# UZ-SLAMLab/DefSLAM

Measured on AMD Instinct MI355X. Metric: SfT GN iters/sec (500-node mesh, 1k matches), higher is better.
Workload: dtype f64

## Files before the change

### defslam_amd/csrc/sft_batch.h

```cpp
#pragma once

#define SFTB_NW 8
#ifndef SFTB_LIN_NW
#define SFTB_LIN_NW 8
#endif
#ifndef SFTB_LIN_WAVES
#define SFTB_LIN_WAVES 2
#endif
#ifndef SFTB_TRIAL_WAVES
#define SFTB_TRIAL_WAVES 2
#endif

__device__ __forceinline__ void sftb_ctl_lds(char* smem, Ctl*& ctl, double*& red, double*& out, double*& panel) {
  ctl = reinterpret_cast<Ctl*>(smem);
  red = reinterpret_cast<double*>(smem + 512);
  out = red + 16 * 27 + 5;
  panel = out + 32;
}

__global__ __launch_bounds__(64 * SFTB_NW, 2) void sftb_init_kernel(const SftDev* __restrict__ probs, SftRun* __restrict__ runs, int* __restrict__ counters, int* __restrict__ lin_list, int tail_below) {
  const SftDev& P = probs[blockIdx.x];
  if (blockIdx.x == 0 && threadIdx.x == 0 && (int)gridDim.x <= tail_below) counters[6] = 1;
  init_state<64 * SFTB_NW>(P);
  if (threadIdx.x == 0) {
// ... 48 lines not shown
    const int b = __builtin_amdgcn_readfirstlane(next_b);
    if (b < 0) break;
    if (tid == 0) { nxt = fetch(); atomicAdd(&counters[9], 1); }
    sftb_lin_problem<NW>(probs[b], runs[b], ctl, red, out, panel);
  }
}

__global__ __launch_bounds__(64, 1) void sftb_factor_kernel(const SftDev* __restrict__ probs, SftRun* __restrict__ runs, int* __restrict__ counters, int B) {
  extern __shared__ __attribute__((aligned(16))) char smem[];
  lds_double* lds = to_lds(reinterpret_cast<double*>(smem));
  const int lane = threadIdx.x;
  if (counters[6]) return;
  for (int i = lane; i < WV_LDS_DOUBLES; i += 64) lds[i] = 0.0;
  if (blockIdx.x == 0 && lane == 0) { counters[2] = 0; counters[3] = 0; }
  WvPrev Q;
  Q.Lg = nullptr; Q.Linv = nullptr; Q.x = nullptr; Q.nT = 0; Q.active = 0; Q.xb = 0.0;
  int n_done = 0;
  while (true) {
    int b = 0;
    if (lane == 0) b = atomicAdd(&counters[1], 1);
    b = __builtin_amdgcn_readfirstlane(b);
    if (b >= B) break;
    if (runs[b].state != SFTB_TRIAL) continue;
    const SftDev& P = probs[b];
    const double lambda = runs[b].lambda;
    double xcam;
    const int ok = wv_factor(P, lambda, lambda, lds, Q, xcam);
    if (lane == 0) runs[b].fact_ok = ok;
    Q = wv_prev_of(P, ok, xcam, lane);
    n_done++;
  }
  int lane_now;
  asm volatile("v_mbcnt_lo_u32_b32 %0, -1, 0\n\tv_mbcnt_hi_u32_b32 %0, -1, %0" : "=v"(lane_now));
  if (Q.active) wv_backsub_now(Q, lane_now);
  if (lane_now == 0 && n_done) atomicAdd(&counters[8], n_done);
}

template <int NW>
__device__ __forceinline__ int sftb_trial_problem(const SftDev& P, SftRun& R, Ctl* ctl, double* red, double* out, double* panel, int* counters, int* lin_list, int b) {
  constexpr int NT = 64 * NW;
  const int tid = threadIdx.x;
  const int Dn = P.Dn;
  const int Dnp = ((Dn + NB - 1) / NB) * NB;
  const int ok = R.fact_ok;
  const double lam = R.lambda;
  const bool in_lds = P.lds_class >= 1;
  if (!in_lds)
    for (int i = tid; i < 3 * P.n; i += NT) {
      const double v = P.xyz[i];
      P.xyz_bak[i] = v;
      const int a = P.act[i / 3];
      if (a >= 0) P.xyz[i] = v + P.x[3 * a + (i % 3)];
    }
  if (tid < 7) R.pose_bak[tid] = P.pose[tid];
  __syncthreads();
  if (tid == 0) pose_oplus(P.pose, P.x + Dnp);
  double sc = 0.0;
  for (int r = tid; r < Dn; r += NT) { const double xv = P.x[r]; sc += xv * (lam * xv + P.Hbord[(size_t)6 * Dnp + r]); }
  if (tid < 6) { const double xv = P.x[Dnp + tid]; sc += xv * (lam * xv + P.Hcorner[42 + tid]); }
  __syncthreads();
  block_sum<1>(&sc, red, out);
  const double scale = out[0];
  __syncthreads();
  const auto staged = asm_records<NW, 1>(P, panel);
  const double chi_new = in_lds ? eval_edges<false, 1>(P, ctl, red, out, staged, P.x)
                                : eval_edges<false, 0>(P, ctl, red, out, asm_records<NW, 0>(P, panel));
  if (tid == 0) {
// ... 133 lines not shown
```

### defslam_amd/csrc/sft_wave.h

```cpp
#pragma once

#if defined(WV_STEP_TRACE) && defined(DSH_LAB)
#define WV_T_DECL long long wv_tr[9] = {0, 0, 0, 0, 0, 0, 0, 0, 0}, wv_tl = clock64()
#define WV_T(e) do { const long long t__ = clock64(); wv_tr[e] += t__ - wv_tl; wv_tl = t__; } while (0)
#define WV_T_ARG , long long (&wv_tr)[9], long long& wv_tl
#define WV_T_PASS , wv_tr, wv_tl
#define WV_T_DUMP(P) do { if ((threadIdx.x & 63) == 0) for (int e__ = 0; e__ < 9; e__++) (P).dbg[40 + e__] = (double)wv_tr[e__]; } while (0)
#else
#define WV_T_DECL do {} while (0)
#define WV_T(e) do {} while (0)
#define WV_T_ARG
#define WV_T_PASS
#define WV_T_DUMP(P) do {} while (0)
#endif

__host__ __device__ constexpr int wv_phys(int r, int d) {
  return d == 0 ? r : (d <= 3 ? 8 * d + r : (d == 4 ? 32 + (r & 3) : 8 * (8 - d) + ((r + 8 - d) & 7)));
}
constexpr int WV_AGPR_TILES = 32;
constexpr int WV_L_WIN = 0;
constexpr int WV_L_BORD = 1024;
constexpr int WV_L_WSCR = 2048;
constexpr int WV_L_CN = 2336;
constexpr int WV_L_XRING = 2400;
constexpr int WV_L_LAND = 2528;
constexpr int WV_LDS_DOUBLES = WV_L_LAND + 10 * 256;
typedef double v2d_w __attribute__((ext_vector_type(2)));
#ifndef WV_DMA_AUX
#define WV_DMA_AUX 0
#endif
using lds_v2d = __attribute__((address_space(3))) v2d_w;

#define WV_NOP_MFMA_RESULT "s_nop 15\n\ts_nop 3"

template <int T>
__device__ __forceinline__ void wv_upd_agpr(const v4d& A, const v4d& B, int q0 = 0) {
  static_assert(T >= 0 && T < WV_AGPR_TILES, "accumulator tile");
#define WV_MF(q) asm volatile("v_mfma_f64_16x16x4_f64 a[%c0:%c1], %2, %3, a[%c0:%c1] neg:[1,0,0]" ::"i"(8 * T), "i"(8 * T + 7), "v"(A[q]), "v"(B[q]) : "memory")
  if (q0 <= 0) WV_MF(0);
  if (q0 <= 1) WV_MF(1);
  if (q0 <= 2) WV_MF(2);
  WV_MF(3);
#undef WV_MF
}
__device__ __forceinline__ void wv_upd_vgpr(v4d& C, const v4d& A, const v4d& B, int q0 = 0) {
#define WV_MF(q) asm volatile("v_mfma_f64_16x16x4_f64 %0, %1, %2, %0 neg:[1,0,0]" : "+v"(C) : "v"(A[q]), "v"(B[q]) : "memory")
  asm volatile("s_nop 1" : "+v"(C));
  if (q0 <= 0) WV_MF(0);
  if (q0 <= 1) WV_MF(1);
  if (q0 <= 2) WV_MF(2);
  WV_MF(3);
#undef WV_MF
}
template <int T>
__device__ __forceinline__ void wv_trsm_agpr(v4d& Y, const v4d& Wt) {
  asm volatile("v_mfma_f64_16x16x4_f64 %0, %1, a[%c5:%c6], 0\n\t"
               "v_mfma_f64_16x16x4_f64 %0, %2, a[%c7:%c8], %0\n\t"
               "v_mfma_f64_16x16x4_f64 %0, %3, a[%c9:%c10], %0\n\t"
               "v_mfma_f64_16x16x4_f64 %0, %4, a[%c11:%c12], %0"
               : "=&v"(Y)
               : "v"(Wt[0]), "v"(Wt[1]), "v"(Wt[2]), "v"(Wt[3]), "i"(8 * T), "i"(8 * T + 1), "i"(8 * T + 2), "i"(8 * T + 3), "i"(8 * T + 4), "i"(8 * T + 5),
                 "i"(8 * T + 6), "i"(8 * T + 7)
               : "memory");
}
__device__ __forceinline__ void wv_trsm_vgpr(v4d& Y, const v4d& Wt, const v4d& D, int q0 = 0) {
  if (q0 <= 0) {
    asm volatile("s_nop 1\n\t"
                 "v_mfma_f64_16x16x4_f64 %0, %1, %5, 0\n\t"
                 "v_mfma_f64_16x16x4_f64 %0, %2, %6, %0\n\t"
                 "v_mfma_f64_16x16x4_f64 %0, %3, %7, %0\n\t"
                 "v_mfma_f64_16x16x4_f64 %0, %4, %8, %0"
                 : "=&v"(Y)
                 : "v"(Wt[0]), "v"(Wt[1]), "v"(Wt[2]), "v"(Wt[3]), "v"(D[0]), "v"(D[1]), "v"(D[2]), "v"(D[3])
                 : "memory");
  } else {
    asm volatile("s_nop 1\n\tv_mfma_f64_16x16x4_f64 %0, %1, %2, 0" : "=&v"(Y) : "v"(Wt[3]), "v"(D[3]) : "memory");
    if (q0 <= 2) asm volatile("v_mfma_f64_16x16x4_f64 %0, %1, %2, %0" : "+v"(Y) : "v"(Wt[2]), "v"(D[2]) : "memory");
    if (q0 <= 1) asm volatile("v_mfma_f64_16x16x4_f64 %0, %1, %2, %0" : "+v"(Y) : "v"(Wt[1]), "v"(D[1]) : "memory");
  }
}
struct WvTri { double a[10]; };
__device__ __forceinline__ void wv_tri_load(const lds_double* wscr, int lane, WvTri& A) {
  const lds_double* p = wscr + (lane & 3) * 17 + (lane >> 4);
#pragma unroll
  for (int q = 0; q < 4; q++)
// ... 90 lines not shown
__device__ __forceinline__ void wv_bq_store(lds_double* tile, int lane, const WvB2& v) {
  reinterpret_cast<lds_v2d*>(tile)[lane] = (v2d_w){v.n0, v.n1};
}
__device__ __forceinline__ int wv_bo_lane(int lane) { return (lane & 0x30) | (lane & 3); }
__device__ __forceinline__ void wv_bo_load(const lds_double* tile, int lane, WvBO& o) {
  const lds_v2d* p = reinterpret_cast<const lds_v2d*>(tile) + wv_bo_lane(lane);
#pragma unroll
  for (int q = 0; q < 4; q++) { const v2d_w a = p[4 * q]; o.v[q][0] = a.x; o.v[q][1] = a.y; }
}
__device__ __forceinline__ void wv_upd_b4(WvB2& C, const v4d& A, const WvBO& B, int q0 = 0) {
#define WV_MF(q) asm volatile("v_mfma_f64_4x4x4_4b_f64 %0, %2, %3, %0 neg:[1,0,0]\n\tv_mfma_f64_4x4x4_4b_f64 %1, %2, %4, %1 neg:[1,0,0]" \
                              : "+v"(C.n0), "+v"(C.n1) : "v"(A[q]), "v"(B.v[q][0]), "v"(B.v[q][1]) : "memory")
  asm volatile("s_nop 1" : "+v"(C.n0), "+v"(C.n1));
  if (q0 <= 0) WV_MF(0);
  if (q0 <= 1) WV_MF(1);
  if (q0 <= 2) WV_MF(2);
  WV_MF(3);
#undef WV_MF
}
__device__ __forceinline__ void wv_trsm_b4(WvB2& Y, const v4d& Wt, const WvBO& B) {
  asm volatile("s_nop 1\n\t"
               "v_mfma_f64_4x4x4_4b_f64 %0, %2, %6, 0\n\t"
               "v_mfma_f64_4x4x4_4b_f64 %1, %2, %7, 0\n\t"
               "v_mfma_f64_4x4x4_4b_f64 %0, %3, %8, %0\n\t"
               "v_mfma_f64_4x4x4_4b_f64 %1, %3, %9, %1\n\t"
               "v_mfma_f64_4x4x4_4b_f64 %0, %4, %10, %0\n\t"
               "v_mfma_f64_4x4x4_4b_f64 %1, %4, %11, %1\n\t"
               "v_mfma_f64_4x4x4_4b_f64 %0, %5, %12, %0\n\t"
               "v_mfma_f64_4x4x4_4b_f64 %1, %5, %13, %1"
               : "=&v"(Y.n0), "=&v"(Y.n1)
               : "v"(Wt[0]), "v"(Wt[1]), "v"(Wt[2]), "v"(Wt[3]), "v"(B.v[0][0]), "v"(B.v[0][1]), "v"(B.v[1][0]), "v"(B.v[1][1]), "v"(B.v[2][0]), "v"(B.v[2][1]),
                 "v"(B.v[3][0]), "v"(B.v[3][1])
               : "memory");
}
__device__ __forceinline__ int wv_bstd_index(int lane) { return 2 * wv_bo_lane(lane) + ((lane >> 2) & 1); }

template <int CTRL>
__device__ __forceinline__ double wv_dpp_mov(double v) {
  const int lo = __builtin_amdgcn_mov_dpp(__double2loint(v), CTRL, 0xF, 0xF, false);
  const int hi = __builtin_amdgcn_mov_dpp(__double2hiint(v), CTRL, 0xF, 0xF, false);
  return __hiloint2double(hi, lo);
}

__device__ __forceinline__ bool wv_chol_inv(v4d& a, v4d& w) {
  const int lane = threadIdx.x & 63;
  const int g = lane >> 4, c = lane & 15;
  w = (v4d){(g == c) ? 1.0 : 0.0, (g + 4 == c) ? 1.0 : 0.0, (g + 8 == c) ? 1.0 : 0.0, (g + 12 == c) ? 1.0 : 0.0};
  double plast = 1.0;
#pragma unroll
  for (int J = 0; J < 4; J++) {
    const double aJ = a[J];
    const double sel = chol4_inverse_operand(aJ, J, g, c & 3, plast);
    const double wJ = w[J];
    double zw, lp;
    if (J < 3) {
      asm volatile("s_nop 1\n\t"
                   "v_mfma_f64_4x4x4_4b_f64 %0, %2, %3, 0\n\t"
                   "v_mfma_f64_4x4x4_4b_f64 %1, %2, %4, 0\n\t"
                   "s_nop 7"
                   : "=&v"(zw), "=&v"(lp)
                   : "v"(sel), "v"(wJ), "v"(aJ));
      const double nlp = -lp;
      const double below = (c >= 4 * J + 4) ? nlp : 0.0;
      asm volatile("s_nop 1\n\t"
                   "v_mfma_f64_16x16x4_f64 %0, %2, %3, %0\n\t"
                   "v_mfma_f64_16x16x4_f64 %1, %4, %5, %1\n\t" WV_NOP_MFMA_RESULT
                   : "+v"(a), "+v"(w)
                   : "v"(nlp), "v"(lp), "v"(below), "v"(zw));
      w[J] = zw;
    } else {
      asm volatile("s_nop 1\n\tv_mfma_f64_4x4x4_4b_f64 %0, %1, %2, 0\n\ts_nop 7" : "=&v"(zw) : "v"(sel), "v"(wJ));
      w[J] = zw;
    }
  }
// ... 54 lines not shown
};
__device__ __forceinline__ void wv_bs_request(const WvPrev& Q, int J, lds_double* land, int lane) {
  const unsigned voff = 16u * (unsigned)lane;
  const SFT_G char* col = reinterpret_cast<const SFT_G char*>(Q.Lg + ((size_t)J * (BT + 1)) * 256);
  const SFT_G char* w = reinterpret_cast<const SFT_G char*>(Q.Linv + (size_t)J * 256);
  const unsigned l0 = (unsigned)__builtin_amdgcn_readfirstlane((int)(size_t)land);
  asm volatile("s_mov_b32 m0, %2\n\ts_nop 0\n\t"
               "global_load_lds_dwordx4 %0, %1\n\t"
               "global_load_lds_dwordx4 %0, %1 offset:2048\n\t"
               "global_load_lds_dwordx4 %0, %1 offset:3072"
               :: "v"(voff), "s"(col), "s"(l0) : "memory", "m0");
#pragma unroll
  for (int grp = 1; grp < 5; grp++) {
    const SFT_G char* cg = col + 4096 * grp;
    const unsigned lg = l0 + 4096u * grp;
    if (grp < 4)
      asm volatile("s_mov_b32 m0, %2\n\ts_nop 0\n\t"
                   "global_load_lds_dwordx4 %0, %1\n\t"
                   "global_load_lds_dwordx4 %0, %1 offset:1024\n\t"
                   "global_load_lds_dwordx4 %0, %1 offset:2048\n\t"
                   "global_load_lds_dwordx4 %0, %1 offset:3072"
                   :: "v"(voff), "s"(cg), "s"(lg) : "memory", "m0");
    else
      asm volatile("s_mov_b32 m0, %2\n\ts_nop 0\n\t"
                   "global_load_lds_dwordx4 %0, %1\n\t"
                   "global_load_lds_dwordx4 %0, %1 offset:1024"
                   :: "v"(voff), "s"(cg), "s"(lg) : "memory", "m0");
  }
  asm volatile("s_mov_b32 m0, %2\n\ts_nop 0\n\t"
               "global_load_lds_dwordx4 %0, %1\n\t"
               "global_load_lds_dwordx4 %0, %1 offset:1024"
               :: "v"(voff), "s"(w), "s"(l0 + 18u * 1024u) : "memory", "m0");
}
__device__ __forceinline__ void wv_bs_column(const WvPrev& Q, int J, const lds_double* land, lds_double* xring, int lane) {
  const int c = lane & 15;
  const lds_v2d* t2 = reinterpret_cast<const lds_v2d*>(land) + 2 * lane;
  double s[4];
  {
    const lds_double* tb = land + wv_bstd_index(lane);
    s[0] = tb[0] * Q.xb; s[1] = tb[8] * Q.xb; s[2] = tb[16] * Q.xb; s[3] = tb[24] * Q.xb;
  }
#pragma unroll
  for (int d = 1; d <= 8; d++) {
    const double xr = xring[((J + d) & 7) * 16 + c];
    const v2d_w a = t2[128 * d], b = t2[128 * d + 1];
    s[0] = fma(a.x, xr, s[0]); s[1] = fma(a.y, xr, s[1]); s[2] = fma(b.x, xr, s[2]); s[3] = fma(b.y, xr, s[3]);
  }
#pragma unroll
  for (int q = 0; q < 4; q++) {
    s[q] += wv_dpp_mov<0x128>(s[q]);
    s[q] += wv_dpp_mov<0x124>(s[q]);
    s[q] += wv_dpp_mov<0x122>(s[q]);
    s[q] += wv_dpp_mov<0x121>(s[q]);
  }
  const v2d_w wa = t2[128 * 9], wb = t2[128 * 9 + 1];
  double p = wa.x * -s[0];
  p = fma(wa.y, -s[1], p); p = fma(wb.x, -s[2], p); p = fma(wb.y, -s[3], p);
  p = sum_rows(p);
  if (lane < TS) { xring[(J & 7) * 16 + lane] = p; Q.x[TS * J + lane] = p; }
}
__device__ __forceinline__ void wv_bs_step(const WvPrev& Q, int J, lds_double* lds, int lane) {
  wv_bs_column(Q, J, lds + WV_L_LAND, lds + WV_L_XRING, lane);
  asm volatile("s_waitcnt lgkmcnt(0)" ::: "memory");
  if (J >= 1) wv_bs_request(Q, J - 1, lds + WV_L_LAND, lane);
}
__device__ __forceinline__ void wv_bs_begin(const WvPrev& Q, lds_double* lds, int lane) {
  lds_double* xring = lds + WV_L_XRING;
  xring[lane] = 0.0; xring[64 + lane] = 0.0;
  wv_bs_request(Q, Q.nT - 1, lds + WV_L_LAND, lane);
}
__device__ __forceinline__ void wv_backsub_now(const WvPrev& Q, int lane) {
  const int c = lane & 15;
  (void)c;
  double xr[8];
#pragma unroll
  for (int s = 0; s < 8; s++) xr[s] = 0.0;
  struct Col { v4d t[10]; };
  auto fetch = [&](int J) -> Col {
    Col C;
    if (J >= 0) {
      const SFT_G double* col = Q.Lg + ((size_t)J * (BT + 1)) * 256 + 4 * lane;
#pragma unroll
      for (int i = 1; i <= 8; i++) C.t[i] = (J + i < Q.nT) ? *reinterpret_cast<const SFT_G v4d*>(col + 256 * i) : (v4d){0.0, 0.0, 0.0, 0.0};
      {
        const SFT_G double* tb = col - 4 * lane + wv_bstd_index(lane);
        C.t[0] = (v4d){tb[0], tb[8], tb[16], tb[24]};
      }
      C.t[9] = *reinterpret_cast<const SFT_G v4d*>(Q.Linv + (size_t)J * 256 + 4 * lane);
    } else {
#pragma unroll
      for (int i = 0; i < 10; i++) C.t[i] = (v4d){0.0, 0.0, 0.0, 0.0};
    }
    return C;
  };
  auto solve_col = [&](const Col& C, int J, auto phc) {
    constexpr int ph = decltype(phc)::value;
    double s[4];
#pragma unroll
    for (int q = 0; q < 4; q++) s[q] = C.t[0][q] * Q.xb;
#pragma unroll
    for (int dd = 1; dd <= 8; dd++)
#pragma unroll
      for (int q = 0; q < 4; q++) s[q] = fma(C.t[dd][q], xr[(ph + dd) & 7], s[q]);
#pragma unroll
    for (int q = 0; q < 4; q++) {
      s[q] += wv_dpp_mov<0x128>(s[q]);
      s[q] += wv_dpp_mov<0x124>(s[q]);
      s[q] += wv_dpp_mov<0x122>(s[q]);
      s[q] += wv_dpp_mov<0x121>(s[q]);
    }
    double p = C.t[9][0] * -s[0];
#pragma unroll
    for (int q = 1; q < 4; q++) p = fma(C.t[9][q], -s[q], p);
    p = sum_rows(p);
    xr[ph] = p;
    if (lane < TS) Q.x[TS * J + lane] = p;
  };
  int J = Q.nT - 1;
  Col c0 = fetch(J), c1 = fetch(J - 1);
#pragma unroll 1
  for (; J >= 0; J -= 2) {
    const Col n0 = fetch(J - 2), n1 = fetch(J - 3);
    switch (J & 7) {
      case 7: solve_col(c0, J, std::integral_constant<int, 7>{}); solve_col(c1, J - 1, std::integral_constant<int, 6>{}); break;
      case 5: solve_col(c0, J, std::integral_constant<int, 5>{}); solve_col(c1, J - 1, std::integral_constant<int, 4>{}); break;
      case 3: solve_col(c0, J, std::integral_constant<int, 3>{}); solve_col(c1, J - 1, std::integral_constant<int, 2>{}); break;
      default: solve_col(c0, J, std::integral_constant<int, 1>{}); solve_col(c1, J - 1, std::integral_constant<int, 0>{}); break;
    }
    c0 = n0; c1 = n1;
  }
}

struct WvState {
  v4d Y[9];
  WvB2 Yq;
  WvBO Yo;
  double corner;
  v4d araw;
  WvB2 bnext;
  WvRowList rl;
  unsigned al[4];
  unsigned off_lane, off_bord;
  int ok;
};

template <int PH, int I, int IEND>
__device__ __forceinline__ void wv_trsm_cols(WvState& S, const WvTri& Wt, int k, int nT, const v4d& D4, int lane) {
  if constexpr (I <= IEND) {
    (void)k; (void)nT;
    if constexpr (I == 4) {
      wv_trsm4_vgpr(S.Y[4], Wt, D4);
    } else {
      wv_trsm4_agpr<wv_phys((PH + I) & 7, I)>(S.Y[I], Wt);
    }
    wv_trsm_cols<PH, I + 1, IEND>(S, Wt, k, nT, D4, lane);
  }
}

__host__ __device__ constexpr int wv_tile_index(int I, int J) {
  int n = 0;
  for (int i = 1; i <= 7; i++)
    for (int j = 1; j <= i; j++) {
// ... 36 lines not shown
  }
}
template <int PH, bool TAIL, int I0, int I1>
__device__ __forceinline__ void wv_update_rows(const WvProb& W, WvState& S, int k, int nT, int q8, SFT_G double* col) {
  if constexpr (I0 <= I1) {
    wv_update_tiles<PH, TAIL, I0, 1>(W, S, k, nT, q8, col);
    wv_update_rows<PH, TAIL, I0 + 1, I1>(W, S, k, nT, q8, col);
  }
}
template <int PH, int T>
__device__ __forceinline__ lds_double* wv_task_tile(lds_double* lds) {
  if constexpr (T < 7) return lds + WV_L_BORD + 128 * ((PH + T + 1) & 7);
  else if constexpr (T < 10) return lds + WV_L_WIN + 256 * (wv_phys((PH + T - 2) & 7, 4) - WV_AGPR_TILES);
  else if constexpr (T == 10) return lds + WV_L_BORD + 128 * (PH & 7);
  else return lds + WV_L_WIN + 256 * (wv_phys(PH & 7, 4) - WV_AGPR_TILES);
}
template <int T> struct WvTaskTile { using type = typename std::conditional<(T < 7 || T == 10), WvB2, v4d>::type; };
template <int T> using wv_task_t = typename WvTaskTile<T>::type;
template <int PH, int T>
__device__ __forceinline__ wv_task_t<T> wv_task_load(lds_double* lds, int lane) {
  if constexpr (T < 7 || T == 10) return wv_bq_load(wv_task_tile<PH, T>(lds), lane);
  else return wv_lds_load(wv_task_tile<PH, T>(lds), lane);
}
template <int PH, int T>
__device__ __forceinline__ void wv_task_store(lds_double* lds, int lane, const wv_task_t<T>& C) {
  if constexpr (T < 7 || T == 10) wv_bq_store(wv_task_tile<PH, T>(lds), lane, C);
  else wv_lds_store(wv_task_tile<PH, T>(lds), lane, C);
}
template <int T>
__device__ __forceinline__ void wv_task_mfma(wv_task_t<T>& C, const WvState& S, int q8) {
  if constexpr (T < 7) wv_upd_b4(C, S.Y[T + 1], S.Yo);
  else if constexpr (T < 10) wv_upd_vgpr(C, S.Y[T - 6], S.Y[T - 2]);
  else if constexpr (T == 10) wv_upd_b4(C, S.Y[8], S.Yo, q8);
  else wv_upd_vgpr(C, S.Y[4], S.Y[8], q8);
}
template <int PH, int T, int TEND>
__device__ __forceinline__ void wv_lds_pipe_next(const WvState& S, int q8, lds_double* lds, int lane, wv_task_t<T>& C, const wv_task_t<T - 1>& Cprev) {
  if constexpr (T < TEND) {
    wv_task_t<T + 1> Cn = wv_task_load<PH, T + 1>(lds, lane);
    wv_task_mfma<T>(C, S, q8);
    wv_task_store<PH, T - 1>(lds, lane, Cprev);
    wv_lds_pipe_next<PH, T + 1, TEND>(S, q8, lds, lane, Cn, C);
  } else {
    wv_task_mfma<T>(C, S, q8);
    wv_task_store<PH, T - 1>(lds, lane, Cprev);
    wv_mfma_fence();
    wv_task_store<PH, T>(lds, lane, C);
  }
}
template <int PH, int T0, int TEND>
__device__ __forceinline__ void wv_lds_pipe(const WvState& S, int q8, lds_double* lds, int lane) {
  wv_task_t<T0> C = wv_task_load<PH, T0>(lds, lane);
  wv_task_t<T0 + 1> Cn = wv_task_load<PH, T0 + 1>(lds, lane);
  wv_task_mfma<T0>(C, S, q8);
  wv_lds_pipe_next<PH, T0 + 1, TEND>(S, q8, lds, lane, Cn, C);
}

template <int PH>
__device__ __forceinline__ v4d wv_step_diag(const WvProb& W, int k, int lane) {
  v4d d = wv_read_agpr<wv_phys(PH, 0)>();
  const int g = lane >> 4, c = lane & 15;
#pragma unroll
  for (int q = 0; q < 4; q++)
    if (g + 4 * q == c && TS * k + c < W.Dn) d[q] += W.lambda;
  return d;
}

template <int PH, bool TAIL>
__device__ __forceinline__ void wv_step_rest(const WvProb& W, WvState& S, const v4d& w, int k, lds_double* lds, int lane, const WvPrev& Q WV_T_ARG) {
  lds_double* ldsw = lds + WV_L_WIN;
  lds_double* ldsb = lds + WV_L_BORD;
  lds_double* wscr = lds + WV_L_WSCR;
  const int nT = W.nT;
  WvBO Bk;
  wv_bo_load(ldsb + 128 * PH, lane, Bk);
  const v4d D4 = wv_lds_load(ldsw + 256 * (wv_phys((PH + 4) & 7, 4) - WV_AGPR_TILES), lane);
  v4d Wt;
  {
    const int g = lane >> 4, c = lane & 15;
#pragma unroll
    for (int q = 0; q < 4; q++) wscr[(g + 4 * q) * 17 + c] = w[q];
#pragma unroll
    for (int q = 0; q < 4; q++) Wt[q] = wscr[c * 17 + g + 4 * q];
  }
  WvTri Wq;
  wv_tri_load(wscr, lane, Wq);
  WV_T(2);
  wv_trsm_b4(S.Yq, Wt, Bk);
  wv_trsm_cols<PH, 1, 2>(S, Wq, k, nT, D4, lane);
// ... 4 lines not shown
  {
    const lds_double* t = wscr + 2 * wv_bo_lane(lane);
    const lds_double* ta = t + (lane >> 3 & 1);
    const lds_double* tb = t + (lane >> 2 & 1);
#pragma unroll
    for (int q = 0; q < 4; q++) { yba[q] = ta[8 * q]; ybs[q] = tb[8 * q]; }
  }
  asm volatile("" :: "v"(D4[0]), "v"(D4[1]), "v"(D4[2]), "v"(D4[3]));
  wv_trsm_cols<PH, 5, 7>(S, Wq, k, nT, D4, lane);
  if (W.q8 == 1) wv_trsm4_vgpr_q1(S.Y[8], Wq, S.araw);
  else wv_trsm_vgpr(S.Y[8], Wt, S.araw, W.q8);
  wv_mfma_fence();
  WV_T(3);
  SFT_G double* col = W.Lg + ((size_t)k * (BT + 1)) * 256;
  v4d fresh4 = wv_gather_vgpr(W, S.rl.o[4]);
  asm volatile("" : "+v"(S.bnext.n0), "+v"(S.bnext.n1));
  wv_bq_store(ldsb + 128 * PH, lane, S.bnext);
  WV_T(4);
  asm volatile("s_nop 1\n\t"
               "v_mfma_f64_4x4x4_4b_f64 %0, %1, %5, %0 neg:[1,0,0]\n\ts_nop 3\n\t"
               "v_mfma_f64_4x4x4_4b_f64 %0, %2, %6, %0 neg:[1,0,0]\n\ts_nop 3\n\t"
               "v_mfma_f64_4x4x4_4b_f64 %0, %3, %7, %0 neg:[1,0,0]\n\ts_nop 3\n\t"
               "v_mfma_f64_4x4x4_4b_f64 %0, %4, %8, %0 neg:[1,0,0]"
               : "+v"(S.corner)
               : "v"(yba[0]), "v"(yba[1]), "v"(yba[2]), "v"(yba[3]), "v"(ybs[0]), "v"(ybs[1]), "v"(ybs[2]), "v"(ybs[3])
               : "memory");
  wv_update_rows<PH, TAIL, 1, 7>(W, S, k, nT, W.q8, col);
  wv_lds_pipe<PH, 0, 9>(S, W.q8, lds, lane);
  WV_T(5);
  wv_wait_vm();
  WV_T(6);
  {
    WvB2 C10 = wv_task_load<PH, 10>(lds, lane);
    wv_update_rows<PH, TAIL, 8, 8>(W, S, k, nT, W.q8, col);
    wv_task_mfma<10>(C10, S, W.q8);
    wv_task_mfma<11>(fresh4, S, W.q8);
    wv_task_store<PH, 10>(lds, lane, C10);
    wv_mfma_fence();
    wv_task_store<PH, 11>(lds, lane, fresh4);
  }
  asm volatile("" : "+v"(S.corner));
  WV_T(8);
}

struct WvTriList { unsigned o[36][4]; };
template <int R, int D>
__device__ __forceinline__ void wv_prologue_lists(const WvProb& W, int lane, WvTriList& T) {
  if constexpr (R < 8) {
    wv_list(W, R, D, lane, T.o[R * (R + 1) / 2 + D]);
    if constexpr (D < R) wv_prologue_lists<R, D + 1>(W, lane, T);
    else wv_prologue_lists<R + 1, 0>(W, lane, T);
  }
}
template <int R, int D>
__device__ __forceinline__ void wv_prologue_gathers(const WvProb& W, WvTriList& T, v4d (&f4)[8]) {
  if constexpr (R < 8) {
    unsigned (&o)[4] = T.o[R * (R + 1) / 2 + D];
    if constexpr (R == 0 && D == 0) {
#pragma unroll
      for (int t = 0; t < 36; t++) asm volatile("" : "+v"(T.o[t][0]), "+v"(T.o[t][1]), "+v"(T.o[t][2]), "+v"(T.o[t][3]));
    }
    if constexpr (D == 4) f4[R] = wv_gather_vgpr(W, o);
    else wv_gather_agpr<wv_phys(R, D)>(W.Hc, o[0], o[1], o[2], o[3]);
    if constexpr (D < R) wv_prologue_gathers<R, D + 1>(W, T, f4);
    else wv_prologue_gathers<R + 1, 0>(W, T, f4);
  }
}
template <int PH>
__device__ __forceinline__ void wv_prologue_store(lds_double* lds, int lane, v4d& f4, WvB2& bd) {
  if constexpr (PH >= 4) {
// ... 43 lines not shown
    wv_prologue_store<0>(lds, lane, f4[0], bd[0]); wv_prologue_store<1>(lds, lane, f4[1], bd[1]); wv_prologue_store<2>(lds, lane, f4[2], bd[2]);
    wv_prologue_store<3>(lds, lane, f4[3], bd[3]); wv_prologue_store<4>(lds, lane, f4[4], bd[4]); wv_prologue_store<5>(lds, lane, f4[5], bd[5]);
    wv_prologue_store<6>(lds, lane, f4[6], bd[6]); wv_prologue_store<7>(lds, lane, f4[7], bd[7]);
  }
  wv_wait_vm();
  asm volatile("" : "+v"(S.al[0]), "+v"(S.al[1]), "+v"(S.al[2]), "+v"(S.al[3]));
#ifdef DSH_LAB
  const long long wv_t1 = clock64();
  const long long wv_w1 = wall_clock64();
#endif

  WV_T_DECL;
#pragma unroll 1
  for (int k = 0; k < W.nT; k++) {
    const int ph = k & 7;
    asm volatile("v_lshlrev_b32 %0, 5, %1" : "=v"(S.off_lane) : "v"(lane));
    asm volatile("v_lshlrev_b32 %0, 4, %1" : "=v"(S.off_bord) : "v"(lane));
    S.araw = wv_gather_vgpr(W, S.al);
    wv_list(W, k + 9, 8, lane, S.al);
    wv_row_list(W, k + 8, lane, S.rl);
    S.bnext = wv_border_fresh(W, k + 8, lane);
    v4d d;
    switch (ph) {
      case 0: d = wv_step_diag<0>(W, k, lane); break;
      case 1: d = wv_step_diag<1>(W, k, lane); break;
      case 2: d = wv_step_diag<2>(W, k, lane); break;
      case 3: d = wv_step_diag<3>(W, k, lane); break;
      case 4: d = wv_step_diag<4>(W, k, lane); break;
      case 5: d = wv_step_diag<5>(W, k, lane); break;
      case 6: d = wv_step_diag<6>(W, k, lane); break;
      default: d = wv_step_diag<7>(W, k, lane); break;
    }
    WV_T(0);
    if (Q.active) {
      const int J = Q.nT - 1 - k;
      if (J >= 0) wv_bs_step(Q, J, lds, lane);
    }
    WV_T(7);
    v4d w;
    if (!wv_chol_inv(d, w)) {
#ifdef DSH_LAB
      if (S.ok && lane == 0) P.dbg[3] = 1000.0 + k;
#endif
      S.ok = 0;
    }
    WV_T(1);
    {
      const SFT_G double* slot = W.Linv + (size_t)k * 256;
      const v2d_w w01 = (v2d_w){w[0], w[1]}, w23 = (v2d_w){w[2], w[3]};
      asm volatile("global_store_dwordx4 %0, %1, %3\n\tglobal_store_dwordx4 %0, %2, %3 offset:16" :: "v"(S.off_lane), "v"(w01), "v"(w23), "s"(slot) : "memory");
    }
    switch (ph + ((k + 8 >= W.nT) ? 8 : 0)) {
      case 0: wv_step_rest<0, false>(W, S, w, k, lds, lane, Q WV_T_PASS); break;
      case 1: wv_step_rest<1, false>(W, S, w, k, lds, lane, Q WV_T_PASS); break;
      case 2: wv_step_rest<2, false>(W, S, w, k, lds, lane, Q WV_T_PASS); break;
      case 3: wv_step_rest<3, false>(W, S, w, k, lds, lane, Q WV_T_PASS); break;
      case 4: wv_step_rest<4, false>(W, S, w, k, lds, lane, Q WV_T_PASS); break;
      case 5: wv_step_rest<5, false>(W, S, w, k, lds, lane, Q WV_T_PASS); break;
      case 6: wv_step_rest<6, false>(W, S, w, k, lds, lane, Q WV_T_PASS); break;
      case 7: wv_step_rest<7, false>(W, S, w, k, lds, lane, Q WV_T_PASS); break;
      case 8: wv_step_rest<0, true>(W, S, w, k, lds, lane, Q WV_T_PASS); break;
      case 9: wv_step_rest<1, true>(W, S, w, k, lds, lane, Q WV_T_PASS); break;
      case 10: wv_step_rest<2, true>(W, S, w, k, lds, lane, Q WV_T_PASS); break;
      case 11: wv_step_rest<3, true>(W, S, w, k, lds, lane, Q WV_T_PASS); break;
      case 12: wv_step_rest<4, true>(W, S, w, k, lds, lane, Q WV_T_PASS); break;
      case 13: wv_step_rest<5, true>(W, S, w, k, lds, lane, Q WV_T_PASS); break;
      case 14: wv_step_rest<6, true>(W, S, w, k, lds, lane, Q WV_T_PASS); break;
      default: wv_step_rest<7, true>(W, S, w, k, lds, lane, Q WV_T_PASS); break;
    }
  }
  WV_T_DUMP(P);
  if (Q.active) {
    for (int J = Q.nT - 1 - W.nT; J >= 0; J--) { wv_wait_vm(); wv_bs_step(Q, J, lds, lane); }
  }
#ifdef DSH_LAB
  const long long wv_t2 = clock64();
  const long long wv_w2 = wall_clock64();
#endif
  wv_mfma_fence();
  {
    int l2;
    asm volatile("v_mbcnt_lo_u32_b32 %0, -1, 0\n\tv_mbcnt_hi_u32_b32 %0, -1, %0" : "=v"(l2));
    const int g2 = l2 >> 4, c2 = l2 & 15;
    const int cr2 = 4 * (c2 >> 3) + g2, cc2 = 4 * ((c2 >> 2) & 1) + (c2 & 3);
    if (cr2 < SFT_BORDER && cc2 < SFT_BORDER) Cn[cr2 * 7 + cc2] = S.corner;
  }
  double xcam = 0.0;
  {
    int okc = 1;
    if (lane == 0) {
      double xc[6] = {0, 0, 0, 0, 0, 0};
      bool bad = false;
      for (int kk = 0; kk < 6; kk++) {
        double dd = Cn[kk * 7 + kk];
        for (int j = 0; j < kk; j++) dd -= Cn[kk * 7 + j] * Cn[kk * 7 + j];
        if (!(dd > 0.0)) bad = true;
        const double piv = sqrt(dd);
        Cn[kk * 7 + kk] = piv;
        for (int r = kk + 1; r < 7; r++) {
          double v = Cn[r * 7 + kk];
          for (int j = 0; j < kk; j++) v -= Cn[r * 7 + j] * Cn[kk * 7 + j];
          Cn[r * 7 + kk] = v / piv;
        }
      }
      if (bad) okc = 0;
      for (int kk = 5; kk >= 0; kk--) {
// ... 10 lines not shown
  xcam_out = xcam;
#ifdef DSH_LAB
  if (lane == 0) { P.dbg[5] = (double)(wv_t1 - wv_t0); P.dbg[6] = (double)(wv_t2 - wv_t1); P.dbg[4] = (double)(wv_w2 - wv_w1); }
#endif
  return __builtin_amdgcn_readfirstlane(S.ok);
}

__device__ __forceinline__ WvPrev wv_prev_of(const SftDev& P, int ok, double xcam, int lane_) {
  (void)lane_;
  int lane;
  asm volatile("v_mbcnt_lo_u32_b32 %0, -1, 0\n\tv_mbcnt_hi_u32_b32 %0, -1, %0" : "=v"(lane));
  const int c = lane & 15;
  WvPrev Q;
  const int Dn = uni(P.Dn), Dnp = ((Dn + NB - 1) / NB) * NB;
  Q.Lg = uni(P.Lb); Q.Linv = uni(P.Linv); Q.x = uni(P.x);
  Q.nT = Dnp / TS;
  Q.active = ok;
  Q.xb = (c < 6) ? xcam : ((c == 6) ? -1.0 : 0.0);
  if (ok && lane < 6) P.x[Dnp + lane] = xcam;
  return Q;
}

__device__ __forceinline__ int wv_factor_solve(const SftDev& P, double lambda, double lam_corner, lds_double* lds) {
  WvPrev none;
  none.Lg = nullptr; none.Linv = nullptr; none.x = nullptr; none.nT = 0; none.active = 0; none.xb = 0.0;
  double xcam;
  const int ok = wv_factor(P, lambda, lam_corner, lds, none, xcam);
  int lane;
  asm volatile("v_mbcnt_lo_u32_b32 %0, -1, 0\n\tv_mbcnt_hi_u32_b32 %0, -1, %0" : "=v"(lane));
  const WvPrev Q = wv_prev_of(P, ok, xcam, lane);
#ifdef DSH_LAB
  const long long t2 = clock64();
#endif
  if (ok) wv_backsub_now(Q, lane);
#ifdef DSH_LAB
  if (lane == 0) P.dbg[7] = (double)(clock64() - t2);
#endif
  return ok;
}
```

Measured before the change: 422,900.

## Move back-substitution onto 4x4 f64 MFMAs and interleave it with factor update rows

```diff
diff --git a/defslam_amd/csrc/sft_batch.h b/defslam_amd/csrc/sft_batch.h
--- a/defslam_amd/csrc/sft_batch.h
+++ b/defslam_amd/csrc/sft_batch.h
@@ -104,7 +104,7 @@
   }
   int lane_now;
   asm volatile("v_mbcnt_lo_u32_b32 %0, -1, 0\n\tv_mbcnt_hi_u32_b32 %0, -1, %0" : "=v"(lane_now));
-  if (Q.active) wv_backsub_now(Q, lane_now);
+  if (Q.active) wv_backsub_now(Q, lds, lane_now);
   if (lane_now == 0 && n_done) atomicAdd(&counters[8], n_done);
 }
 
diff --git a/defslam_amd/csrc/sft_wave.h b/defslam_amd/csrc/sft_wave.h
--- a/defslam_amd/csrc/sft_wave.h
+++ b/defslam_amd/csrc/sft_wave.h
@@ -51,6 +51,19 @@
   if (q0 <= 2) WV_MF(2);
   WV_MF(3);
 #undef WV_MF
+}
+__device__ __forceinline__ void wv_upd_vgpr_q(v4d& C, const v4d& A, const v4d& B, int q0) {
+#define WV_UQ(body) \
+  asm volatile("s_nop 1\n\t" body "\n\t" WV_NOP_MFMA_RESULT : "+v"(C) : "v"(A[0]), "v"(A[1]), "v"(A[2]), "v"(A[3]), "v"(B[0]), "v"(B[1]), "v"(B[2]), "v"(B[3]) : "memory")
+#define WV_MQ(a, b) "v_mfma_f64_16x16x4_f64 %0, %" #a ", %" #b ", %0 neg:[1,0,0]"
+  switch (q0) {
+    case 0: WV_UQ(WV_MQ(1, 5) "\n\t" WV_MQ(2, 6) "\n\t" WV_MQ(3, 7) "\n\t" WV_MQ(4, 8)); break;
+    case 1: WV_UQ(WV_MQ(2, 6) "\n\t" WV_MQ(3, 7) "\n\t" WV_MQ(4, 8)); break;
+    case 2: WV_UQ(WV_MQ(3, 7) "\n\t" WV_MQ(4, 8)); break;
+    default: WV_UQ(WV_MQ(4, 8)); break;
+  }
+#undef WV_MQ
+#undef WV_UQ
 }
 template <int T>
 __device__ __forceinline__ void wv_trsm_agpr(v4d& Y, const v4d& Wt) {
@@ -207,14 +220,6 @@
                : "v"(Wt[0]), "v"(Wt[1]), "v"(Wt[2]), "v"(Wt[3]), "v"(B.v[0][0]), "v"(B.v[0][1]), "v"(B.v[1][0]), "v"(B.v[1][1]), "v"(B.v[2][0]), "v"(B.v[2][1]),
                  "v"(B.v[3][0]), "v"(B.v[3][1])
                : "memory");
-}
-__device__ __forceinline__ int wv_bstd_index(int lane) { return 2 * wv_bo_lane(lane) + ((lane >> 2) & 1); }
-
-template <int CTRL>
-__device__ __forceinline__ double wv_dpp_mov(double v) {
-  const int lo = __builtin_amdgcn_mov_dpp(__double2loint(v), CTRL, 0xF, 0xF, false);
-  const int hi = __builtin_amdgcn_mov_dpp(__double2hiint(v), CTRL, 0xF, 0xF, false);
-  return __hiloint2double(hi, lo);
 }
 
 __device__ __forceinline__ bool wv_chol_inv(v4d& a, v4d& w) {
@@ -335,102 +340,136 @@
                "global_load_lds_dwordx4 %0, %1 offset:1024"
                :: "v"(voff), "s"(w), "s"(l0 + 18u * 1024u) : "memory", "m0");
 }
-__device__ __forceinline__ void wv_bs_column(const WvPrev& Q, int J, const lds_double* land, lds_double* xring, int lane) {
-  const int c = lane & 15;
-  const lds_v2d* t2 = reinterpret_cast<const lds_v2d*>(land) + 2 * lane;
-  double s[4];
-  {
-    const lds_double* tb = land + wv_bstd_index(lane);
-    s[0] = tb[0] * Q.xb; s[1] = tb[8] * Q.xb; s[2] = tb[16] * Q.xb; s[3] = tb[24] * Q.xb;
-  }
-#pragma unroll
-  for (int d = 1; d <= 8; d++) {
-    const double xr = xring[((J + d) & 7) * 16 + c];
-    const v2d_w a = t2[128 * d], b = t2[128 * d + 1];
-    s[0] = fma(a.x, xr, s[0]); s[1] = fma(a.y, xr, s[1]); s[2] = fma(b.x, xr, s[2]); s[3] = fma(b.y, xr, s[3]);
-  }
-#pragma unroll
-  for (int q = 0; q < 4; q++) {
-    s[q] += wv_dpp_mov<0x128>(s[q]);
-    s[q] += wv_dpp_mov<0x124>(s[q]);
-    s[q] += wv_dpp_mov<0x122>(s[q]);
-    s[q] += wv_dpp_mov<0x121>(s[q]);
-  }
-  const v2d_w wa = t2[128 * 9], wb = t2[128 * 9 + 1];
-  double p = wa.x * -s[0];
-  p = fma(wa.y, -s[1], p); p = fma(wb.x, -s[2], p); p = fma(wb.y, -s[3], p);
-  p = sum_rows(p);
-  if (lane < TS) { xring[(J & 7) * 16 + lane] = p; Q.x[TS * J + lane] = p; }
-}
-__device__ __forceinline__ void wv_bs_step(const WvPrev& Q, int J, lds_double* lds, int lane) {
-  wv_bs_column(Q, J, lds + WV_L_LAND, lds + WV_L_XRING, lane);
+__device__ __forceinline__ void wv_bs_request_lds(const WvPrev& Q, int J, lds_double* lds, int lane) {
   asm volatile("s_waitcnt lgkmcnt(0)" ::: "memory");
-  if (J >= 1) wv_bs_request(Q, J - 1, lds + WV_L_LAND, lane);
+  wv_bs_request(Q, J, lds + WV_L_LAND, lane);
+}
+
+constexpr int WV_L_BSS = WV_L_LAND + 128;
+constexpr int WV_L_BSXB = WV_L_LAND + 144;
+__device__ __forceinline__ int wv_bs_ta(int lane) { return 64 * (lane & 3) + 4 * (lane >> 4) + ((lane >> 2) & 3); }
+__device__ __forceinline__ int wv_bs_tb(int lane) { return 32 * (lane & 3) + 8 * ((lane >> 2) & 3) + 2 * (lane >> 4); }
+__device__ __forceinline__ v4d wv_bs_bl(const lds_double* v, int lane) {
+  const lds_v2d* p = reinterpret_cast<const lds_v2d*>(v + 4 * (lane >> 4));
+  const v2d_w a = p[0], b = p[1];
+  return (v4d){a.x, a.y, b.x, b.y};
+}
+__device__ __forceinline__ void wv_bs_mf_yb(double& s0, double& s1, const v2d_w& a, const v2d_w& b) {
+  asm volatile("s_nop 1\n\t"
+               "v_mfma_f64_4x4x4_4b_f64 %0, %2, %4, 0\n\t"
+               "v_mfma_f64_4x4x4_4b_f64 %1, %3, %5, 0"
+               : "=&v"(s0), "=&v"(s1)
+               : "v"(a.x), "v"(a.y), "v"(b.x), "v"(b.y)
+               : "memory");
+}
+__device__ __forceinline__ void wv_bs_mf_tile(double& s0, double& s1, const v4d& a, const v4d& b) {
+  asm volatile("s_nop 1\n\t"
+               "v_mfma_f64_4x4x4_4b_f64 %0, %2, %6, %0\n\t"
+               "v_mfma_f64_4x4x4_4b_f64 %1, %3, %7, %1\n\t"
+               "v_mfma_f64_4x4x4_4b_f64 %0, %4, %8, %0\n\t"
+               "v_mfma_f64_4x4x4_4b_f64 %1, %5, %9, %1"
+               : "+v"(s0), "+v"(s1)
+               : "v"(a[0]), "v"(a[1]), "v"(a[2]), "v"(a[3]), "v"(b[0]), "v"(b[1]), "v"(b[2]), "v"(b[3])
+               : "memory");
+}
+__device__ __forceinline__ void wv_bs_mf_w(double& x0, double& x1, const v4d& sb, const v4d& w) {
+  asm volatile("s_nop 1\n\t"
+               "v_mfma_f64_4x4x4_4b_f64 %0, %2, %6, 0 neg:[1,0,0]\n\t"
+               "v_mfma_f64_4x4x4_4b_f64 %1, %3, %7, 0 neg:[1,0,0]\n\t"
+               "v_mfma_f64_4x4x4_4b_f64 %0, %4, %8, %0 neg:[1,0,0]\n\t"
+               "v_mfma_f64_4x4x4_4b_f64 %1, %5, %9, %1 neg:[1,0,0]"
+               : "=&v"(x0), "=&v"(x1)
+               : "v"(sb[0]), "v"(sb[1]), "v"(sb[2]), "v"(sb[3]), "v"(w[0]), "v"(w[1]), "v"(w[2]), "v"(w[3])
+               : "memory");
+}
+__device__ __forceinline__ double wv_bs_sum(double s0, double s1) {
+  asm volatile("s_nop 8" : "+v"(s0), "+v"(s1));
+  return s0 + s1;
+}
+struct WvBsLds {
+  const lds_double* land;
+  int ta, tb, lane;
+  __device__ __forceinline__ v2d_w yb() const { return *reinterpret_cast<const lds_v2d*>(land + tb); }
+  template <int D>
+  __device__ __forceinline__ v4d tile() const { const lds_double* p = land + 256 * D + ta; return (v4d){p[0], p[16], p[32], p[48]}; }
+  __device__ __forceinline__ v4d w() const {
+    const lds_v2d* p = reinterpret_cast<const lds_v2d*>(land + 256 * 9) + 2 * lane;
+    const v2d_w a = p[0], b = p[1];
+    return (v4d){a.x, a.y, b.x, b.y};
+  }
+};
+__device__ __forceinline__ WvBsLds wv_bs_lds(lds_double* lds, int lane) { return WvBsLds{lds + WV_L_LAND, wv_bs_ta(lane), wv_bs_tb(lane), lane}; }
+struct WvBsCol { v2d_w yb; v4d t[8]; v4d w; };
+__device__ __forceinline__ void wv_bs_fetch(const WvPrev& Q, int J, int lane, WvBsCol& C) {
+  const SFT_G double* col = Q.Lg + ((size_t)J * (BT + 1)) * 256;
+  C.yb = *reinterpret_cast<const SFT_G v2d_w*>(col + wv_bs_tb(lane));
+  const SFT_G double* p = col + wv_bs_ta(lane);
+#pragma unroll
+  for (int d = 1; d <= 8; d++) C.t[d - 1] = (v4d){p[256 * d], p[256 * d + 16], p[256 * d + 32], p[256 * d + 48]};
+  C.w = *reinterpret_cast<const SFT_G v4d*>(Q.Linv + (size_t)J * 256 + 4 * lane);
+}
+struct WvBsRegs {
+  const WvBsCol& C;
+  __device__ __forceinline__ v2d_w yb() const { return C.yb; }
+  template <int D>
+  __device__ __forceinline__ v4d tile() const { return C.t[D - 1]; }
+  __device__ __forceinline__ v4d w() const { return C.w; }
+};
+struct WvBsSepNop {
+  template <int D>
+  __device__ __forceinline__ void run() const { if constexpr (D <= 8) asm volatile("s_nop 7" ::: "memory"); }
+  template <int D>
+  __device__ __forceinline__ void pin() const {}
+};
+template <int D, class Src, class Sep>
+__device__ __forceinline__ void wv_bs_pipe(double& s0, double& s1, const Src& src, const Sep& sep, const lds_double* xring, int slot, int lane,
+                                           const v2d_w& yb, const v2d_w& xb, const v4d& a, const v4d& b, v4d& w) {
+  sep.template run<D>();
+  if constexpr (D < 8) {
+    const v4d an = src.template tile<D + 1>(), bn = wv_bs_bl(xring + 16 * ((slot - D - 1) & 7), lane);
+    sep.template pin<D>();
+    if constexpr (D == 1) wv_bs_mf_yb(s0, s1, yb, xb);
+    wv_bs_mf_tile(s0, s1, a, b);
+    wv_bs_pipe<D + 1>(s0, s1, src, sep, xring, slot, lane, yb, xb, an, bn, w);
+  } else {
+    w = src.w();
+    sep.template pin<D>();
+    wv_bs_mf_tile(s0, s1, a, b);
+  }
+}
+template <class Src, class Sep>
+__device__ __forceinline__ void wv_bs_col(const WvPrev& Q, int J, int slot, lds_double* lds, int lane, const Src& src, const Sep& sep) {
+  lds_double* xring = lds + WV_L_XRING;
+  const v2d_w yb = src.yb(), xb = reinterpret_cast<const lds_v2d*>(lds + WV_L_BSXB)[lane >> 4];
+  const v4d a1 = src.template tile<1>(), b1 = wv_bs_bl(xring + 16 * ((slot - 1) & 7), lane);
+  double s0, s1;
+  v4d w;
+  wv_bs_pipe<1>(s0, s1, src, sep, xring, slot, lane, yb, xb, a1, b1, w);
+  const double S = wv_bs_sum(s0, s1);
+  lds[WV_L_BSS + 4 * (lane >> 4) + ((lane >> 2) & 3)] = S;
+  const v4d sb = wv_bs_bl(lds + WV_L_BSS, lane);
+  sep.template run<9>();
+  double x0, x1;
+  wv_bs_mf_w(x0, x1, sb, w);
+  const double x = wv_bs_sum(x0, x1);
+  if (lane < TS) { xring[16 * (slot & 7) + 4 * (lane & 3) + (lane >> 2)] = x; Q.x[TS * J + lane] = x; }
 }
 __device__ __forceinline__ void wv_bs_begin(const WvPrev& Q, lds_double* lds, int lane) {
   lds_double* xring = lds + WV_L_XRING;
   xring[lane] = 0.0; xring[64 + lane] = 0.0;
-  wv_bs_request(Q, Q.nT - 1, lds + WV_L_LAND, lane);
-}
-__device__ __forceinline__ void wv_backsub_now(const WvPrev& Q, int lane) {
-  const int c = lane & 15;
-  (void)c;
-  double xr[8];
-#pragma unroll
-  for (int s = 0; s < 8; s++) xr[s] = 0.0;
-  struct Col { v4d t[10]; };
-  auto fetch = [&](int J) -> Col {
-    Col C;
-    if (J >= 0) {
-      const SFT_G double* col = Q.Lg + ((size_t)J * (BT + 1)) * 256 + 4 * lane;
-#pragma unroll
-      for (int i = 1; i <= 8; i++) C.t[i] = (J + i < Q.nT) ? *reinterpret_cast<const SFT_G v4d*>(col + 256 * i) : (v4d){0.0, 0.0, 0.0, 0.0};
-      {
-        const SFT_G double* tb = col - 4 * lane + wv_bstd_index(lane);
-        C.t[0] = (v4d){tb[0], tb[8], tb[16], tb[24]};
-      }
-      C.t[9] = *reinterpret_cast<const SFT_G v4d*>(Q.Linv + (size_t)J * 256 + 4 * lane);
-    } else {
-#pragma unroll
-      for (int i = 0; i < 10; i++) C.t[i] = (v4d){0.0, 0.0, 0.0, 0.0};
-    }
-    return C;
-  };
-  auto solve_col = [&](const Col& C, int J, auto phc) {
-    constexpr int ph = decltype(phc)::value;
-    double s[4];
-#pragma unroll
-    for (int q = 0; q < 4; q++) s[q] = C.t[0][q] * Q.xb;
-#pragma unroll
-    for (int dd = 1; dd <= 8; dd++)
-#pragma unroll
-      for (int q = 0; q < 4; q++) s[q] = fma(C.t[dd][q], xr[(ph + dd) & 7], s[q]);
-#pragma unroll
-    for (int q = 0; q < 4; q++) {
-      s[q] += wv_dpp_mov<0x128>(s[q]);
-      s[q] += wv_dpp_mov<0x124>(s[q]);
-      s[q] += wv_dpp_mov<0x122>(s[q]);
-      s[q] += wv_dpp_mov<0x121>(s[q]);
-    }
-    double p = C.t[9][0] * -s[0];
-#pragma unroll
-    for (int q = 1; q < 4; q++) p = fma(C.t[9][q], -s[q], p);
-    p = sum_rows(p);
-    xr[ph] = p;
-    if (lane < TS) Q.x[TS * J + lane] = p;
-  };
-  int J = Q.nT - 1;
-  Col c0 = fetch(J), c1 = fetch(J - 1);
+  if (lane < 8) lds[WV_L_BSXB + 2 * (lane & 3) + (lane >> 2)] = Q.xb;
+}
+__device__ __forceinline__ void wv_backsub_now(const WvPrev& Q, lds_double* lds, int lane) {
+  wv_bs_begin(Q, lds, lane);
+  const WvBsSepNop sep;
+  WvBsCol c0, c1;
+  wv_bs_fetch(Q, Q.nT - 1, lane, c0);
 #pragma unroll 1
-  for (; J >= 0; J -= 2) {
-    const Col n0 = fetch(J - 2), n1 = fetch(J - 3);
-    switch (J & 7) {
-      case 7: solve_col(c0, J, std::integral_constant<int, 7>{}); solve_col(c1, J - 1, std::integral_constant<int, 6>{}); break;
-      case 5: solve_col(c0, J, std::integral_constant<int, 5>{}); solve_col(c1, J - 1, std::integral_constant<int, 4>{}); break;
-      case 3: solve_col(c0, J, std::integral_constant<int, 3>{}); solve_col(c1, J - 1, std::integral_constant<int, 2>{}); break;
-      default: solve_col(c0, J, std::integral_constant<int, 1>{}); solve_col(c1, J - 1, std::integral_constant<int, 0>{}); break;
-    }
-    c0 = n0; c1 = n1;
+  for (int J = Q.nT - 1; J >= 1; J -= 2) {
+    wv_bs_fetch(Q, J - 1, lane, c1);
+    wv_bs_col(Q, J, (Q.nT - 1 - J) & 7, lds, lane, WvBsRegs{c0}, sep);
+    if (J >= 2) wv_bs_fetch(Q, J - 2, lane, c0);
+    wv_bs_col(Q, J - 1, (Q.nT - J) & 7, lds, lane, WvBsRegs{c1}, sep);
   }
 }
 
@@ -533,7 +572,7 @@
   if constexpr (T < 7) wv_upd_b4(C, S.Y[T + 1], S.Yo);
   else if constexpr (T < 10) wv_upd_vgpr(C, S.Y[T - 6], S.Y[T - 2]);
   else if constexpr (T == 10) wv_upd_b4(C, S.Y[8], S.Yo, q8);
-  else wv_upd_vgpr(C, S.Y[4], S.Y[8], q8);
+  else wv_upd_vgpr_q(C, S.Y[4], S.Y[8], q8);
 }
 template <int PH, int T, int TEND>
 __device__ __forceinline__ void wv_lds_pipe_next(const WvState& S, int q8, lds_double* lds, int lane, wv_task_t<T>& C, const wv_task_t<T - 1>& Cprev) {
@@ -556,6 +595,39 @@
   wv_task_mfma<T0>(C, S, q8);
   wv_lds_pipe_next<PH, T0 + 1, TEND>(S, q8, lds, lane, Cn, C);
 }
+
+template <int PH, bool TAIL>
+struct WvBsSepRow8 {
+  WvState& S;
+  v4d& fresh4;
+  WvB2& C10;
+  int q8;
+  lds_double* lds;
+  int lane;
+  template <int D>
+  __device__ __forceinline__ void run() const {
+    if constexpr (D <= 7) {
+      constexpr int J = D < 4 ? D : D + 1;
+      if constexpr (TAIL) asm volatile("s_nop 7" ::: "memory");
+      else wv_upd_agpr<wv_phys(PH, 8 - J)>(S.Y[J], S.Y[8], q8);
+    } else if constexpr (D == 8) {
+      wv_task_mfma<10>(C10, S, q8);
+    } else {
+      wv_task_mfma<11>(fresh4, S, q8);
+      wv_task_store<PH, 10>(lds, lane, C10);
+    }
+  }
+  template <int D>
+  __device__ __forceinline__ void pin() const {
+    if constexpr (D <= 7 && !TAIL) {
+      constexpr int J = D < 4 ? D : D + 1;
+      asm volatile("" ::"v"(S.Y[J][0]), "v"(S.Y[J][1]), "v"(S.Y[J][2]), "v"(S.Y[J][3]));
+    } else if constexpr (D == 8) {
+      asm volatile("" ::"v"(S.Yo.v[0][0]), "v"(S.Yo.v[0][1]), "v"(S.Yo.v[1][0]), "v"(S.Yo.v[1][1]), "v"(S.Yo.v[2][0]), "v"(S.Yo.v[2][1]),
+                   "v"(S.Yo.v[3][0]), "v"(S.Yo.v[3][1]));
+    }
+  }
+};
 
 template <int PH>
 __device__ __forceinline__ v4d wv_step_diag(const WvProb& W, int k, int lane) {
@@ -626,10 +698,18 @@
   WV_T(6);
   {
     WvB2 C10 = wv_task_load<PH, 10>(lds, lane);
-    wv_update_rows<PH, TAIL, 8, 8>(W, S, k, nT, W.q8, col);
-    wv_task_mfma<10>(C10, S, W.q8);
-    wv_task_mfma<11>(fresh4, S, W.q8);
-    wv_task_store<PH, 10>(lds, lane, C10);
+    const int J = Q.nT - 1 - k;
+    if (Q.active && J >= 0) {
+      int l2;
+      asm volatile("v_mbcnt_lo_u32_b32 %0, -1, 0\n\tv_mbcnt_hi_u32_b32 %0, -1, %0" : "=v"(l2));
+      const WvBsSepRow8<PH, TAIL> sep{S, fresh4, C10, W.q8, lds, l2};
+      wv_bs_col(Q, J, PH, lds, l2, wv_bs_lds(lds, l2), sep);
+    } else {
+      wv_update_rows<PH, TAIL, 8, 8>(W, S, k, nT, W.q8, col);
+      wv_task_mfma<10>(C10, S, W.q8);
+      wv_task_mfma<11>(fresh4, S, W.q8);
+      wv_task_store<PH, 10>(lds, lane, C10);
+    }
     wv_mfma_fence();
     wv_task_store<PH, 11>(lds, lane, fresh4);
   }
@@ -739,10 +819,7 @@
       default: d = wv_step_diag<7>(W, k, lane); break;
     }
     WV_T(0);
-    if (Q.active) {
-      const int J = Q.nT - 1 - k;
-      if (J >= 0) wv_bs_step(Q, J, lds, lane);
-    }
+    if (Q.active && Q.nT - 1 - k >= 0) wv_bs_request_lds(Q, Q.nT - 1 - k, lds, lane);
     WV_T(7);
     v4d w;
     if (!wv_chol_inv(d, w)) {
@@ -778,7 +855,13 @@
   }
   WV_T_DUMP(P);
   if (Q.active) {
-    for (int J = Q.nT - 1 - W.nT; J >= 0; J--) { wv_wait_vm(); wv_bs_step(Q, J, lds, lane); }
+    int l2;
+    asm volatile("v_mbcnt_lo_u32_b32 %0, -1, 0\n\tv_mbcnt_hi_u32_b32 %0, -1, %0" : "=v"(l2));
+    for (int J = Q.nT - 1 - W.nT; J >= 0; J--) {
+      wv_bs_request_lds(Q, J, lds, l2);
+      wv_wait_vm();
+      wv_bs_col(Q, J, (Q.nT - 1 - J) & 7, lds, l2, wv_bs_lds(lds, l2), WvBsSepNop{});
+    }
   }
 #ifdef DSH_LAB
   const long long wv_t2 = clock64();
@@ -855,7 +938,7 @@
 #ifdef DSH_LAB
   const long long t2 = clock64();
 #endif
-  if (ok) wv_backsub_now(Q, lane);
+  if (ok) wv_backsub_now(Q, lds, lane);
 #ifdef DSH_LAB
   if (lane == 0) P.dbg[7] = (double)(clock64() - t2);
 #endif
```

Result: slower. 400,700, median of 2 (-5.3%).
